# SymbioticLab/Oobleck

Measured on AMD Instinct MI355X. Metric: tokens/sec (whole node) GPT-2 1F1B, higher is better.
Workload: dtype bf16; 1 GPU; gpt2.yaml GPT-2-small 1F1B, global microbatch 128x1024 tokens, bf16; model=gpt2, global_batch=128, seq_len=1024, parallelism=pp1dp1

## Files before the change

include/oobleck_stage.h:

```cpp
#ifndef OOBLECK_STAGE_H
#define OOBLECK_STAGE_H

#include <stdint.h>

#ifdef __cplusplus
extern "C" {
#endif

enum {
  OB_KIND_EMBED = 0,
  OB_KIND_BLOCK = 1,
  OB_KIND_FINAL = 2
};

typedef struct ob_layer* ob_layer_t;

typedef struct {
  int32_t kind;
  int32_t n_embd;
  int32_t n_head;
  int32_t n_positions;
  int32_t vocab_size;
  int32_t max_batch;
  int32_t seq_len;
// ... 96 lines not shown
                    void* stream);
int ob_dropout_scale_f32(uint64_t seed, int32_t layer_id, int32_t site,
                         uint64_t tick, float p, const void* x, void* y,
                         int64_t n, void* stream);
int ob_dropout_scale_bf16(uint64_t seed, int32_t layer_id, int32_t site,
                          uint64_t tick, float p, const void* x, void* y,
                          int64_t n, void* stream);
int ob_dropout_add_f32(uint64_t seed, int32_t layer_id, int32_t site,
                       uint64_t tick, float p, const void* t, const void* res,
                       void* y, int64_t n, void* stream);
int ob_dropout_add_bf16(uint64_t seed, int32_t layer_id, int32_t site,
                        uint64_t tick, float p, const void* t,
                        const void* res, void* y, int64_t n, void* stream);
int ob_dropout_scale_colsum_f32(uint64_t seed, int32_t layer_id, int32_t site,
                                uint64_t tick, float p, const void* dy,
                                void* dm, void* db, int64_t M, int64_t N,
                                void* stream);
int ob_dropout_scale_colsum_bf16(uint64_t seed, int32_t layer_id, int32_t site,
                                 uint64_t tick, float p, const void* dy,
                                 void* dm, void* db, int64_t M, int64_t N,
                                 void* stream);

int ob_gemm_bf16(int transA, int transB, int64_t M, int64_t N, int64_t K,
                 float alpha, const void* A, int64_t lda,
                 int64_t strideA1, int64_t strideA2,
                 const void* B, int64_t ldb,
                 int64_t strideB1, int64_t strideB2,
                 float beta, void* C, int64_t ldc,
                 int64_t strideC1, int64_t strideC2,
                 int64_t n1, int64_t n2,
                 const void* bias, const void* residual, int out_kind,
                 int splitk, void* stream);

int ob_f32_to_bf16(const void* x, void* y, int64_t n, void* stream);
int ob_f32_to_bf16_t(const void* x, void* y, int64_t rows, int64_t cols,
                     void* stream);
int ob_bf16_to_f32(const void* x, void* y, int64_t n, void* stream);

void ob_profile_enable(int on);
void ob_profile_reset(void);
int ob_profile_read(int fam, double* total_ms, long long* count);

const char* ob_last_error(void);

const char* ob_build_arch(void);

#ifdef __cplusplus
}
#endif
#endif
```

oobleck_amd/_ext.py:

```python
from __future__ import annotations

import ctypes
import pathlib

_LIB = None
SO_PATH = pathlib.Path(__file__).resolve().parent / "libob_stage.so"


class ObLayerDesc(ctypes.Structure):
    _fields_ = [
        ("kind", ctypes.c_int32),
        ("n_embd", ctypes.c_int32),
        ("n_head", ctypes.c_int32),
        ("n_positions", ctypes.c_int32),
        ("vocab_size", ctypes.c_int32),
        ("max_batch", ctypes.c_int32),
        ("seq_len", ctypes.c_int32),
        ("n_slots", ctypes.c_int32),
        ("dtype", ctypes.c_int32),
    ]


class ObDropoutDesc(ctypes.Structure):
    _fields_ = [
# ... 78 lines not shown
    lib.ob_gemm_lt_bias.argtypes = [i32, i32, i64, i64, i64, f32, vp, i64,
                                    vp, i64, f32, vp, i64, i32, vp, vp]
    lib.ob_gemm_lt_f32.argtypes = [i32, i32, i64, i64, i64, f32, vp, i64,
                                   vp, i64, f32, vp, i64, vp]
    lib.ob_flash_fwd_bf16.argtypes = [vp, vp, vp, vp, i64, i64, i64, i64,
                                      f32, vp]
    lib.ob_transpose_bf16_b.argtypes = [vp, vp, i64, i64, i64, i64, i64,
                                        i64, i64, vp]
    lib.ob_layernorm_fwd_bf16.argtypes = [vp, vp, vp, vp, vp, vp, i64, i64,
                                          f32, vp]
    lib.ob_layernorm_bwd_bf16.argtypes = [vp, vp, vp, vp, vp, vp, vp, vp,
                                          i64, i64, i32, vp]
    lib.ob_colsum_bf16.argtypes = [vp, vp, i64, i64, vp]
    lib.ob_layernorm_fwd_copy_bf16.argtypes = [vp, vp, vp, vp, vp, vp, vp,
                                               i64, i64, f32, vp]
    lib.ob_layernorm_bwd_res_bf16.argtypes = [vp, vp, vp, vp, vp, vp, vp, vp,
                                              vp, vp, vp, i64, i64, vp]
    lib.ob_gelu_bwd_colsum_bf16.argtypes = [vp, vp, vp, vp, i64, i64, vp]
    lib.ob_gemm_lt.argtypes = [i32, i32, i64, i64, i64, f32, vp, i64, vp,
                               i64, f32, vp, i64, i32, vp]
    lib.ob_gemm_bf16_nt_8ph.argtypes = [vp, vp, vp, vp, vp, i64, i64, i64,
                                        i64, i64, i64, i64, i64, i64, i64,
                                        i64, i64, i64, i64, f32, f32, i32,
                                        i32, vp, i64]
    lib.ob_profile_enable.argtypes = [i32]
    lib.ob_profile_enable.restype = None
    lib.ob_profile_reset.argtypes = []
    lib.ob_profile_reset.restype = None
    lib.ob_profile_read.argtypes = [i32, ctypes.POINTER(ctypes.c_double),
                                    ctypes.POINTER(ctypes.c_longlong)]
    lib.ob_flash_dsum_bf16.argtypes = [vp, vp, vp, i64, i64, i64, i64, vp]
    lib.ob_flash_bwd_bf16.argtypes = [vp, vp, vp, vp, vp, vp, vp, vp, i64,
                                      i64, i64, i64, f32, vp]
    return lib


def get_ext(build_if_missing: bool = True) -> ctypes.CDLL:
    global _LIB
    if _LIB is not None:
        return _LIB
    if not SO_PATH.exists():
        if build_if_missing:
            from .build import build
            try:
                build()
            except Exception as e:
                raise RuntimeError(
                    f"oobleck_amd: HIP extension missing and build failed: {e}. "
                    "The hot path has no fallback — run __graft_entry__.build().") from e
        else:
            raise RuntimeError(
                "oobleck_amd: HIP extension libob_stage.so is missing. "
                "The hot path has no fallback — run __graft_entry__.build().")
    _LIB = _configure(ctypes.CDLL(str(SO_PATH)))
    return _LIB


def check(rc: int, what: str = "") -> None:
    if rc != 0:
        err = get_ext().ob_last_error().decode()
        raise RuntimeError(f"oobleck_amd extension error in {what}: {err}")
```

oobleck_amd/csrc/ob_internal.h:

```cpp
#pragma once
#include <hip/hip_runtime.h>

#include <cstdarg>
#include <cstdint>
#include <cstdio>

#include "../../include/oobleck_stage.h"

int ob_fail(const char* fmt, ...);

#define OB_HIP(x)                                                     \
  do {                                                                \
    hipError_t e_ = (x);                                              \
    if (e_ != hipSuccess)                                             \
      return ob_fail("%s:%d: %s", __FILE__, __LINE__,                 \
                     hipGetErrorString(e_));                          \
  } while (0)

#define OB_LAUNCH_CHECK()                                             \
  do {                                                                \
    hipError_t e_ = hipGetLastError();                                \
    if (e_ != hipSuccess)                                             \
      return ob_fail("%s:%d: launch: %s", __FILE__, __LINE__,         \
                     hipGetErrorString(e_));                          \
// ... 95 lines not shown
int ob_softmax_causal_bwd_bf16(const void* P, void* dP, int64_t batch,
                               int64_t Sq, void* stream);
int ob_gelu_fwd_bf16(const void* u, void* g, int64_t n, void* stream);
int ob_gelu_bwd_bf16(const void* u, const void* dg, void* du, int64_t n,
                     void* stream);
int ob_colsum_bf16(const void* X, void* db, int64_t M, int64_t N,
                   void* stream);
int ob_embed_fwd_bf16(const void* ids, const void* wte, const void* wpe,
                      void* out, int64_t B, int64_t Sq, int64_t H,
                      void* stream);
int ob_embed_bwd_bf16(const void* ids, const void* dout, void* dwte,
                      void* dwpe, int64_t B, int64_t Sq, int64_t H,
                      void* stream);
int ob_ce_fwd_bf16(const void* logits, const void* labels, void* lse,
                   void* loss, int64_t B, int64_t Sq, int64_t V, int64_t ld,
                   void* stream);
int ob_ce_bwd_bf16(void* logits, const void* labels, const void* lse,
                   const void* dloss, int64_t B, int64_t Sq, int64_t V,
                   int64_t ld, void* stream);
int ob_transpose_bf16(const void* in, void* out, int64_t R, int64_t C,
                      void* stream);
int ob_flash_fwd_bf16(const void* qkv, const void* VT, void* O, void* lse,
                      int64_t B, int64_t Sq, int64_t H, int64_t nh,
                      float scale, void* stream);
int ob_transpose_bf16_b(const void* in, void* out, int64_t R, int64_t C,
                        int64_t sIn1, int64_t sIn2, int64_t ldin, int64_t n1,
                        int64_t n2, void* stream);
int ob_flash_dsum_bf16(const void* O, const void* dO, void* D, int64_t B,
                       int64_t Sq, int64_t H, int64_t nh, void* stream);
int ob_flash_bwd_bf16(const void* qkv, const void* QT, const void* KT,
                      const void* dOT, const void* dO, const void* lse,
                      const void* D, void* dqkv, int64_t B, int64_t Sq,
                      int64_t H, int64_t nh, float scale, void* stream);
}
extern "C" int ob_gemm_lt(int tA, int tB, int64_t M, int64_t N, int64_t K,
                          float alpha, const void* A, int64_t lda,
                          const void* B, int64_t ldb, float beta, void* C,
                          int64_t ldc, int c_f32, void* stream);
extern "C" int ob_gemm_lt_bias(int tA, int tB, int64_t M, int64_t N,
                               int64_t K, float alpha, const void* A,
                               int64_t lda, const void* B, int64_t ldb,
                               float beta, void* C, int64_t ldc, int c_f32,
                               const void* bias, void* stream);
extern "C" int ob_gemm_lt_bias_res(int tA, int tB, int64_t M, int64_t N,
                                   int64_t K, float alpha, const void* A,
                                   int64_t lda, const void* B, int64_t ldb,
                                   void* C, int64_t ldc, int c_f32,
                                   const void* bias, const void* residual,
                                   void* stream);
extern "C" int ob_gemm_lt_f32(int tA, int tB, int64_t M, int64_t N,
                              int64_t K, float alpha, const void* A,
                              int64_t lda, const void* B, int64_t ldb,
                              float beta, void* C, int64_t ldc,
                              void* stream);
extern "C" int ob_gemm_bf16_nt_8ph(const void* A, const void* B, void* C,
                                   const void* bias, const void* residual,
                                   int64_t M, int64_t N, int64_t K,
                                   int64_t lda, int64_t ldb, int64_t ldc,
                                   int64_t sA1, int64_t sA2, int64_t sB1,
                                   int64_t sB2, int64_t sC1, int64_t sC2,
                                   int64_t n1, int64_t n2, float alpha,
                                   float beta, int out_kind, int splitk,
                                   void* stream, int64_t Mr);
int ob_gemm_bf16_nt_dispatch(const void* A, const void* B, void* C,
                             const void* bias, const void* residual,
                             int64_t M, int64_t N, int64_t K, int64_t lda,
// ... 6 lines not shown
```

oobleck_amd/csrc/ob_kernels_bf16.hip:

```cpp
#include "ob_internal.h"

#include <cmath>

using f32x16 = __attribute__((ext_vector_type(16))) float;
using bf16x8 = __attribute__((ext_vector_type(8))) __bf16;

static inline hipStream_t S(void* s) { return reinterpret_cast<hipStream_t>(s); }

#define BF_BM 128
#define BF_BN 128
#define BF_BK 32
#define BF_LDS_K 40

enum { BF_OUT_BF16 = 0, BF_OUT_F32 = 1, BF_OUT_F32_ATOMIC = 2 };

__device__ __forceinline__ float bf2f(__bf16 h) { return (float)h; }

__device__ __forceinline__ unsigned bf_bits(__bf16 h) {
  return (unsigned)__builtin_bit_cast(unsigned short, h);
}
__device__ __forceinline__ __bf16 bits_bf(unsigned u) {
  return __builtin_bit_cast(__bf16, (unsigned short)(u & 0xffffu));
}

// ... 3360 lines not shown
        (const __bf16*)qkv, (const __bf16*)QT, (const __bf16*)dOT,
        (const __bf16*)dO, (const float*)lse, (const float*)D,
        (__bf16*)dqkv, (int)Sq, (int)H, (int)nh, scale);
    OB_LAUNCH_CHECK();
  } else if (dsel == 'p') {
    dim3 gridp((unsigned)(Sq / 64), 1, (unsigned)(B * nh));
    k_flash_bwd_dkdv_p<<<gridp, 256, 0, S(stream)>>>(
        (const __bf16*)qkv, (const __bf16*)QT, (const __bf16*)dOT,
        (const __bf16*)dO, (const float*)lse, (const float*)D,
        (__bf16*)dqkv, (int)Sq, (int)H, (int)nh, scale);
    OB_LAUNCH_CHECK();
  } else {
    k_flash_bwd_dkdv<2><<<grid, 256, 0, S(stream)>>>(
        (const __bf16*)qkv, (const __bf16*)QT, (const __bf16*)dOT,
        (const __bf16*)dO, (const float*)lse, (const float*)D, (__bf16*)dqkv,
        (int)Sq, (int)H, (int)nh, scale);
    OB_LAUNCH_CHECK();
  }
  const char* dqe = getenv("OB_FLASH_DQ");
  if (dqe && dqe[0] == '1')
    k_flash_bwd_dq<<<grid, 256, 0, S(stream)>>>(
        (const __bf16*)qkv, (const __bf16*)KT, (const __bf16*)dO,
        (const float*)lse, (const float*)D, (__bf16*)dqkv, (int)Sq, (int)H,
        (int)nh, scale);
  else
    k_flash_bwd_dq_v3<<<grid, 256, 0, S(stream)>>>(
        (const __bf16*)qkv, (const __bf16*)KT, (const __bf16*)dO,
        (const float*)lse, (const float*)D, (__bf16*)dqkv, (int)Sq, (int)H,
        (int)nh, scale);
  OB_LAUNCH_CHECK();
  return 0;
}


using f32x4 = __attribute__((ext_vector_type(4))) float;

template <int OUT, int SWZ = 0>
__global__ __launch_bounds__(512, 1) void k_gemm_bf16_nt_8ph(
    const __bf16* __restrict__ A, const __bf16* __restrict__ B,
    void* __restrict__ Cv, const float* __restrict__ bias,
    const __bf16* __restrict__ R, int M, int N, int K, int64_t lda,
    int64_t ldb, int64_t ldc, int64_t sA1, int64_t sA2, int64_t sB1,
    int64_t sB2, int64_t sC1, int64_t sC2, int n2, float alpha, float beta,
    int nbn, int Mr) {
  __shared__ __bf16 lds[2][4][128 * 64];

  const int tile = bf_xcd_swz(blockIdx.x, gridDim.x);
  const int bm = tile / nbn, bn = tile % nbn;
  const int m0 = bm * 256, n0 = bn * 256;

  const int z = blockIdx.z;
  const int i1 = z / n2, i2 = z % n2;
  A += (int64_t)i1 * sA1 + (int64_t)i2 * sA2;
  B += (int64_t)i1 * sB1 + (int64_t)i2 * sB2;
  float* Cf = reinterpret_cast<float*>(Cv);
  __bf16* Cb = reinterpret_cast<__bf16*>(Cv);
  const int64_t coff = (int64_t)i1 * sC1 + (int64_t)i2 * sC2;
  Cf += coff;
  Cb += coff;
  if (R) R += coff;

  const int splitk = gridDim.y;
  constexpr int BK = 64;
  const int kchunk = ((K + splitk * BK - 1) / (splitk * BK)) * BK;
  const int kbeg = blockIdx.y * kchunk;
  const int kend = min(K, kbeg + kchunk);
// ... 195 lines not shown
```

oobleck_amd/csrc/ob_layer.hip:

```cpp
#include "ob_internal.h"
#include "ob_philox.h"

#include <cmath>
#include <cstring>
#include <vector>

static inline hipStream_t S(void* s) { return reinterpret_cast<hipStream_t>(s); }
static inline int64_t i64min(int64_t a, int64_t b) { return a < b ? a : b; }
static inline int64_t i64max(int64_t a, int64_t b) { return a > b ? a : b; }


struct Workspace {
  float* dp = nullptr;
  float* bsh1 = nullptr;
  float* bsh2 = nullptr;
  float* dqkv = nullptr;
  float* b4h = nullptr;
  float* t1 = nullptr;
  float* t2 = nullptr;
  float* s1 = nullptr;
  float* s2 = nullptr;
  float* pd_f = nullptr;
  float* pd_b = nullptr;
  float* dm1 = nullptr;
// ... 125 lines not shown
  int64_t o_x = 0, o_mean1 = 0, o_rstd1 = 0, o_ln1 = 0, o_qkv = 0, o_p = 0,
          o_attnm = 0, o_hmid = 0, o_mean2 = 0, o_rstd2 = 0, o_ln2 = 0,
          o_u = 0, o_g = 0, o_logits = 0, o_lse = 0;
  __bf16* shadows = nullptr;
  int64_t v_pad = 0;
  int64_t sh_qkv = 0, sh_qkv_t = 0, sh_ap = 0, sh_ap_t = 0, sh_fc = 0,
          sh_fc_t = 0, sh_mp = 0, sh_mp_t = 0, sh_lm = 0, sh_lm_t = 0;
  int64_t shadow_count = 0;
  bool flash = false;
  float p_embd = 0.f, p_resid = 0.f, p_attn = 0.f;
  int32_t layer_id = 0;
  uint64_t seed = 0;
  bool training = true;
  uint64_t next_tick = 0;
  std::vector<uint8_t> slot_drop;
  std::vector<uint64_t> slot_tick;
};

static bool has_dropout(const ob_layer* l) {
  return l->p_embd > 0.f || l->p_resid > 0.f || l->p_attn > 0.f;
}
static ob_drop_key drop_key(const ob_layer* l, int slot, int site, float p) {
  return ob_drop_make_key(l->seed, l->layer_id, site, l->slot_tick[slot], p);
}

static bool flash_eligible(const ob_layer_desc* d, float attn_pdrop = 0.f) {
  if (attn_pdrop > 0.f) return false;
  static const bool off = [] {
    const char* e = getenv("OB_BF16_FLASH");
    return e && e[0] == '0';
  }();
  return !off && d->dtype == 1 && d->n_embd / d->n_head == 64 &&
         d->seq_len % 128 == 0;
}

struct BlockParams {
  int64_t ln1_w, ln1_b, w_qkv, b_qkv, w_attnproj, b_attnproj, ln2_w, ln2_b,
      w_fc, b_fc, w_mlpproj, b_mlpproj, total;
};
static BlockParams block_params(int64_t H) {
  BlockParams p;
  int64_t o = 0;
  p.ln1_w = o; o += H;
  p.ln1_b = o; o += H;
  p.w_qkv = o; o += H * 3 * H;
  p.b_qkv = o; o += 3 * H;
  p.w_attnproj = o; o += H * H;
  p.b_attnproj = o; o += H;
  p.ln2_w = o; o += H;
  p.ln2_b = o; o += H;
  p.w_fc = o; o += H * 4 * H;
  p.b_fc = o; o += 4 * H;
  p.w_mlpproj = o; o += 4 * H * H;
  p.b_mlpproj = o; o += H;
  p.total = o;
  return p;
}

extern "C" int64_t ob_layer_param_count(const ob_layer_desc* d) {
  const int64_t H = d->n_embd, V = d->vocab_size, P = d->n_positions;
  switch (d->kind) {
    case OB_KIND_EMBED: return V * H + P * H;
    case OB_KIND_BLOCK: return block_params(H).total;
    case OB_KIND_FINAL: return 2 * H + V * H;
  }
  return -1;
// ... 78 lines not shown
      return ob_fail("create: ids hipMalloc failed");
    }
  }
  l->v_pad = (V + 255) / 256 * 256;
  if (d->dtype == 1) {
    int64_t o2 = 0;
    if (d->kind == OB_KIND_BLOCK) {
      l->sh_qkv = o2; o2 += 3 * H * H;
      l->sh_qkv_t = o2; o2 += 3 * H * H;
      l->sh_ap = o2; o2 += H * H;
      l->sh_ap_t = o2; o2 += H * H;
      l->sh_fc = o2; o2 += 4 * H * H;
      l->sh_fc_t = o2; o2 += 4 * H * H;
      l->sh_mp = o2; o2 += 4 * H * H;
      l->sh_mp_t = o2; o2 += 4 * H * H;
    } else if (d->kind == OB_KIND_FINAL) {
      l->sh_lm = o2; o2 += l->v_pad * H;
      l->sh_lm_t = o2; o2 += H * l->v_pad;
    }
    l->shadow_count = o2;
    if (o2 > 0) {
      if (hipMalloc(&l->shadows, (size_t)o2 * sizeof(__bf16)) != hipSuccess)
        return ob_fail("create: shadow hipMalloc failed");
      OB_HIP(hipMemset(l->shadows, 0, (size_t)o2 * sizeof(__bf16)));
    }
  }
  if (d->kind == OB_KIND_BLOCK) {
    if (!l->flash &&
        ws_ensure(&g_ws.dp, &g_ws.sz_dp, Bm * nh * Sq * Sq))
      return 1;
    if (ws_ensure(&g_ws.dqkv, &g_ws.sz_dqkv, BS * 3 * H)) return 1;
    if (ws_ensure(&g_ws.b4h, &g_ws.sz_b4h, BS * 4 * H)) return 1;
    if (d->dtype == 1) {
      if (ws_ensure(&g_ws.t1, &g_ws.sz_t1, (4 * H * BS + 1) / 2)) return 1;
      if (ws_ensure(&g_ws.t2, &g_ws.sz_t2, (4 * H * BS + 1) / 2)) return 1;
      if (ws_ensure(&g_ws.s1, &g_ws.sz_s1, (4 * H * BS + 1) / 2)) return 1;
      if (ws_ensure(&g_ws.s2, &g_ws.sz_s2, (4 * H * BS + 1) / 2)) return 1;
      if (side_init()) return 1;
    }
  }
  if (d->kind == OB_KIND_FINAL && d->dtype == 1) {
    if (ws_ensure(&g_ws.t1, &g_ws.sz_t1, (l->v_pad * BS + 1) / 2)) return 1;
    if (ws_ensure(&g_ws.t2, &g_ws.sz_t2, (4 * H * BS + 1) / 2)) return 1;
    if (ws_ensure(&g_ws.s1, &g_ws.sz_s1, (l->v_pad * BS + 1) / 2)) return 1;
    if (ws_ensure(&g_ws.s2, &g_ws.sz_s2, (4 * H * BS + 1) / 2)) return 1;
    if (side_init()) return 1;
  }
  if (d->kind != OB_KIND_EMBED) {
    const int64_t need = BSH;
    if (ws_ensure(&g_ws.bsh1, &g_ws.sz_bsh, need)) return 1;
    if (ws_ensure(&g_ws.bsh2, &g_ws.sz_bsh2, need)) return 1;
  }
  if (l->p_attn > 0.f) {
    if (ws_ensure(&g_ws.pd_f, &g_ws.sz_pd_f, Bm * nh * Sq * Sq)) return 1;
    if (ws_ensure(&g_ws.pd_b, &g_ws.sz_pd_b, Bm * nh * Sq * Sq)) return 1;
  }
  if (l->p_resid > 0.f) {
    if (ws_ensure(&g_ws.dm1, &g_ws.sz_dm1, BSH)) return 1;
    if (ws_ensure(&g_ws.dm2, &g_ws.sz_dm2, BSH)) return 1;
  }
  *out = l;
  return 0;
}

extern "C" int ob_layer_create(const ob_layer_desc* d, ob_layer_t* out) {
  return layer_create(d, nullptr, out);
}

// ... 267 lines not shown
  return gemm_bf(0, 1, actw, dyw, BS, 1.f, XT, BS, 0, 0, DYT, BS, 0, 0, gout,
                 ldc, 0, 0, 1, 1, nullptr, nullptr, 2,
                 pick_splitk(actw, dyw, BS), stream);
}

static bool use_flash(const ob_layer* l) { return l->flash; }

static int block_forward_bf16(ob_layer* l, int slot, const __bf16* in,
                              __bf16* out, void* stream) {
  const int64_t Sq = l->d.seq_len, H = l->d.n_embd, nh = l->d.n_head;
  const int64_t B = l->B, BS = B * Sq;
  const int64_t hd = H / nh;
  float* st = l->stash + (int64_t)slot * l->slot_stride;
  const float* p = l->params;
  const __bf16* sh = l->shadows;
  const BlockParams bp = block_params(H);
  const bool dA = l->slot_drop[slot] && l->p_attn > 0.f;
  const bool dR = l->slot_drop[slot] && l->p_resid > 0.f;

  __bf16* x = (__bf16*)(st + l->o_x);
  __bf16* ln1 = (__bf16*)(st + l->o_ln1);
  if (OB_PROF(OB_PF_LN, stream,
              ob_layernorm_fwd_copy_bf16(in, p + bp.ln1_w, p + bp.ln1_b, ln1,
                                         x, st + l->o_mean1, st + l->o_rstd1,
                                         BS, H, 1e-5f, stream)))
    return 1;
  __bf16* qkv = (__bf16*)(st + l->o_qkv);
  if (OB_PROF(OB_PF_GEMM_FWD, stream,
              gemm_bf(0, 1, BS, 3 * H, H, 1.f, ln1, H, 0, 0,
                      sh + l->sh_qkv_t, H, 0, 0, qkv, 3 * H, 0, 0, 1, 1,
                      p + bp.b_qkv, nullptr, 0, 1, stream)))
    return 1;
  __bf16* am = (__bf16*)(st + l->o_attnm);
  if (use_flash(l)) {
    __bf16* VTw = (__bf16*)g_ws.t2;
    if (OB_PROF(OB_PF_FLASH_FWD, stream,
                ob_transpose_bf16_b(qkv + 2 * H, VTw, Sq, 64, Sq * 3 * H, 64,
                                    3 * H, B, nh, stream)))
      return 1;
    float* lseP = st + l->o_p;
    if (OB_PROF(OB_PF_FLASH_FWD, stream,
                ob_flash_fwd_bf16(qkv, VTw, am, lseP, B, Sq, H, nh,
                                  1.f / sqrtf((float)hd), stream)))
      return 1;
  } else {
    __bf16* P = (__bf16*)(st + l->o_p);
    if (OB_PROF(OB_PF_ATTN_MAT, stream,
                gemm_bf(0, 1, Sq, Sq, hd, 1.f, qkv, 3 * H, Sq * 3 * H, hd,
                        qkv + H, 3 * H, Sq * 3 * H, hd, P, Sq, nh * Sq * Sq,
                        Sq * Sq, B, nh, nullptr, nullptr, 0, 1, stream)))
      return 1;
    if (OB_PROF(OB_PF_ATTN_MAT, stream,
                ob_softmax_causal_fwd_bf16(P, B * nh, Sq,
                                           1.f / sqrtf((float)hd), stream)))
      return 1;
    const __bf16* Pv = P;
    if (dA) {
      if (OB_PROF(OB_PF_ELEM, stream,
                  ob_drop_scale(drop_key(l, slot, OB_DROP_ATTN, l->p_attn), 1,
                                P, g_ws.pd_f, B * nh * Sq * Sq, stream)))
        return 1;
      Pv = (const __bf16*)g_ws.pd_f;
    }
    if (OB_PROF(OB_PF_ATTN_MAT, stream,
                gemm_bf(0, 0, Sq, hd, Sq, 1.f, Pv, Sq, nh * Sq * Sq, Sq * Sq,
                        qkv + 2 * H, 3 * H, Sq * 3 * H, hd, am, H, Sq * H,
                        hd, B, nh, nullptr, nullptr, 0, 1, stream)))
// ... 137 lines not shown
              gemm_bf(0, 1, BS, H, 4 * H, 1.f, DY4, 4 * H, 0, 0,
                      sh + l->sh_fc, 4 * H, 0, 0, DLN, H, 0, 0, 1, 1,
                      nullptr, nullptr, 0, 1, stream)))
    return 1;
  if (OB_PROF(OB_PF_LN, stream,
              ob_layernorm_bwd_res_bf16(hmid, p + bp.ln2_w, st + l->o_mean2,
                                        st + l->o_rstd2, DLN, dout, din,
                                        g + bp.ln2_w, g + bp.ln2_b,
                                        dR ? nullptr : g + bp.b_mlpproj,
                                        dR ? nullptr : g + bp.b_attnproj,
                                        BS, H, stream)))
    return 1;
  const __bf16* dap = din;
  if (dR) {
    if (OB_PROF(OB_PF_ELEM, stream,
                ob_drop_scale_colsum(
                    drop_key(l, slot, OB_DROP_RESID_ATTN, l->p_resid), 1, din,
                    g_ws.dm1, g + bp.b_attnproj, BS, H, stream)))
      return 1;
    dap = (const __bf16*)g_ws.dm1;
  }
  OB_SIDE_FENCE(S(stream), g_side.stream);
  if (OB_PROF(OB_PF_GEMM_DX, stream,
              gemm_bf(0, 1, BS, H, H, 1.f, dap, H, 0, 0, sh + l->sh_ap, H, 0,
                      0, DATT, H, 0, 0, 1, 1, nullptr, nullptr, 0, 1,
                      stream)))
    return 1;
  if (OB_PROF(OB_PF_GEMM_DW, side,
              dw_bf16_ws(am, H, dap, H, BS, g + bp.w_attnproj, H, g_ws.s1,
                         g_ws.s2, side)))
    return 1;
  hipEvent_t ev_din_done = side_evt();
  OB_HIP(hipEventRecord(ev_din_done, g_side.stream));
  if (use_flash(l)) {
    const int64_t BSH = BS * H;
    __bf16* QTw = (__bf16*)g_ws.t1;
    __bf16* KTw = QTw + BSH;
    __bf16* dOTw = KTw + BSH;
    float* Dbuf = g_ws.t1 + (3 * BSH + 1) / 2;
    const float* lseP = st + l->o_p;
    if (OB_PROF(OB_PF_FLASH_BWD, stream,
                ob_transpose_bf16_b(qkv, QTw, Sq, 64, Sq * 3 * H, 64, 3 * H,
                                    B, nh, stream)))
      return 1;
    if (OB_PROF(OB_PF_FLASH_BWD, stream,
                ob_transpose_bf16_b(qkv + H, KTw, Sq, 64, Sq * 3 * H, 64,
                                    3 * H, B, nh, stream)))
      return 1;
    if (OB_PROF(OB_PF_FLASH_BWD, stream,
                ob_transpose_bf16_b(DATT, dOTw, Sq, 64, Sq * H, 64, H, B, nh,
                                    stream)))
      return 1;
    if (OB_PROF(OB_PF_FLASH_BWD, stream,
                ob_flash_dsum_bf16(am, DATT, Dbuf, B, Sq, H, nh, stream)))
      return 1;
    if (OB_PROF(OB_PF_FLASH_BWD, stream,
                ob_flash_bwd_bf16(qkv, QTw, KTw, dOTw, DATT, lseP, Dbuf,
                                  DQKV, B, Sq, H, nh, scale, stream)))
      return 1;
  } else {
    if (OB_PROF(OB_PF_ATTN_MAT, stream,
                gemm_bf(0, 1, Sq, Sq, hd, 1.f, DATT, H, Sq * H, hd,
                        qkv + 2 * H, 3 * H, Sq * 3 * H, hd, DP, Sq,
                        nh * Sq * Sq, Sq * Sq, B, nh, nullptr, nullptr, 0, 1,
                        stream)))
      return 1;
    const __bf16* Pv = P;
    if (dA) {
      const ob_drop_key ka = drop_key(l, slot, OB_DROP_ATTN, l->p_attn);
      if (OB_PROF(OB_PF_ELEM, stream,
                  ob_drop_scale(ka, 1, P, g_ws.pd_b, B * nh * Sq * Sq,
                                stream)))
        return 1;
      if (OB_PROF(OB_PF_ELEM, stream,
                  ob_drop_scale(ka, 1, DP, DP, B * nh * Sq * Sq, stream)))
        return 1;
      Pv = (const __bf16*)g_ws.pd_b;
    }
    if (OB_PROF(OB_PF_ATTN_MAT, stream,
                ob_softmax_causal_bwd_bf16(P, DP, B * nh, Sq, stream)))
      return 1;
    if (OB_PROF(OB_PF_ATTN_MAT, stream,
                gemm_bf(0, 0, Sq, hd, Sq, scale, DP, Sq, nh * Sq * Sq,
                        Sq * Sq, qkv + H, 3 * H, Sq * 3 * H, hd, DQKV, 3 * H,
                        Sq * 3 * H, hd, B, nh, nullptr, nullptr, 0, 1,
                        stream)))
      return 1;
    if (OB_PROF(OB_PF_ATTN_MAT, stream,
                gemm_bf(1, 0, Sq, hd, Sq, scale, DP, Sq, nh * Sq * Sq,
                        Sq * Sq, qkv, 3 * H, Sq * 3 * H, hd, DQKV + H, 3 * H,
                        Sq * 3 * H, hd, B, nh, nullptr, nullptr, 0, 1,
                        stream)))
      return 1;
    if (OB_PROF(OB_PF_ATTN_MAT, stream,
                gemm_bf(1, 0, Sq, hd, Sq, 1.f, Pv, Sq, nh * Sq * Sq, Sq * Sq,
                        DATT, H, Sq * H, hd, DQKV + 2 * H, 3 * H, Sq * 3 * H,
                        hd, B, nh, nullptr, nullptr, 0, 1, stream)))
      return 1;
  }
  OB_SIDE_FENCE(S(stream), g_side.stream);
  if (OB_PROF(OB_PF_ELEM, side,
              ob_colsum_bf16(DQKV, g + bp.b_qkv, BS, 3 * H, side)))
    return 1;
  if (OB_PROF(OB_PF_GEMM_DW, side,
              dw_bf16_ws(ln1, H, DQKV, 3 * H, BS, g + bp.w_qkv, 3 * H,
                         g_ws.s1, g_ws.s2, side)))
    return 1;
  if (OB_PROF(OB_PF_GEMM_DX, stream,
              gemm_bf(0, 1, BS, H, 3 * H, 1.f, DQKV, 3 * H, 0, 0,
                      sh + l->sh_qkv, 3 * H, 0, 0, DLN, H, 0, 0, 1, 1,
                      nullptr, nullptr, 0, 1, stream)))
    return 1;
  OB_HIP(hipStreamWaitEvent(S(stream), ev_din_done, 0));
  if (OB_PROF(OB_PF_LN, stream,
              ob_layernorm_bwd_bf16(x, p + bp.ln1_w, st + l->o_mean1,
                                    st + l->o_rstd1, DLN, din, g + bp.ln1_w,
                                    g + bp.ln1_b, BS, H, 1, stream)))
    return 1;
  OB_SIDE_FENCE(g_side.stream, S(stream));
  return 0;
}

static int final_backward_bf16(ob_layer* l, int slot, const float* dout,
                               __bf16* din, void* stream) {
  const int64_t Sq = l->d.seq_len, H = l->d.n_embd, V = l->d.vocab_size;
  const int64_t B = l->B, BS = B * Sq;
  float* st = l->stash + (int64_t)slot * l->slot_stride;
  const float* p = l->params;
  float* g = l->grads;
  __bf16* x = (__bf16*)(st + l->o_x);
  __bf16* lnf = (__bf16*)(st + l->o_ln1);
  __bf16* logits = (__bf16*)(st + l->o_logits);
  int64_t* labs = l->ids + (int64_t)slot * (int64_t)l->d.max_batch * Sq;
  __bf16* DLN = (__bf16*)g_ws.bsh1;
// ... 275 lines not shown
```

Before: 639,300 tokens/s.

## Add transpose-free flash attention kernels using LDS transposed reads and fused qkv bias grad

Adds new flash attention forward and backward kernels that read Q, K and V straight from the packed qkv buffer. They stage tiles in swizzled LDS and use ds_read_tr16 transposed loads, so the separate transpose kernels for V, Q, K and dO are no longer needed. The backward kernels also fold the qkv bias gradient column-sum into their epilogues through atomics, which drops the separate colsum launch. The path is on by default and can be turned off with an environment variable. In exchange it adds float atomics on the bias gradient and rebalances the backward work between a dK/dV kernel and a dQ kernel.

```diff
diff --git a/include/oobleck_stage.h b/include/oobleck_stage.h
--- a/include/oobleck_stage.h
+++ b/include/oobleck_stage.h
@@ -152,6 +152,14 @@
                  const void* bias, const void* residual, int out_kind,
                  int splitk, void* stream);
 
+int ob_flash_fwd_nt_bf16(const void* qkv, void* O, void* lse, int64_t B,
+                         int64_t Sq, int64_t H, int64_t nh, float scale,
+                         void* stream);
+int ob_flash_bwd_nt_bf16(const void* qkv, const void* dO, const void* lse,
+                         const void* D, void* dqkv, void* dbias_qkv,
+                         int64_t B, int64_t Sq, int64_t H, int64_t nh,
+                         float scale, void* stream);
+
 int ob_f32_to_bf16(const void* x, void* y, int64_t n, void* stream);
 int ob_f32_to_bf16_t(const void* x, void* y, int64_t rows, int64_t cols,
                      void* stream);
diff --git a/oobleck_amd/_ext.py b/oobleck_amd/_ext.py
--- a/oobleck_amd/_ext.py
+++ b/oobleck_amd/_ext.py
@@ -134,6 +134,10 @@
     lib.ob_flash_dsum_bf16.argtypes = [vp, vp, vp, i64, i64, i64, i64, vp]
     lib.ob_flash_bwd_bf16.argtypes = [vp, vp, vp, vp, vp, vp, vp, vp, i64,
                                       i64, i64, i64, f32, vp]
+    lib.ob_flash_fwd_nt_bf16.argtypes = [vp, vp, vp, i64, i64, i64, i64,
+                                         f32, vp]
+    lib.ob_flash_bwd_nt_bf16.argtypes = [vp, vp, vp, vp, vp, vp, i64, i64,
+                                         i64, i64, f32, vp]
     return lib
 
 
diff --git a/oobleck_amd/csrc/ob_internal.h b/oobleck_amd/csrc/ob_internal.h
--- a/oobleck_amd/csrc/ob_internal.h
+++ b/oobleck_amd/csrc/ob_internal.h
@@ -151,6 +151,13 @@
                       const void* dOT, const void* dO, const void* lse,
                       const void* D, void* dqkv, int64_t B, int64_t Sq,
                       int64_t H, int64_t nh, float scale, void* stream);
+int ob_flash_fwd_nt_bf16(const void* qkv, void* O, void* lse, int64_t B,
+                         int64_t Sq, int64_t H, int64_t nh, float scale,
+                         void* stream);
+int ob_flash_bwd_nt_bf16(const void* qkv, const void* dO, const void* lse,
+                         const void* D, void* dqkv, void* dbias_qkv,
+                         int64_t B, int64_t Sq, int64_t H, int64_t nh,
+                         float scale, void* stream);
 }
 extern "C" int ob_gemm_lt(int tA, int tB, int64_t M, int64_t N, int64_t K,
                           float alpha, const void* A, int64_t lda,
diff --git a/oobleck_amd/csrc/ob_kernels_bf16.hip b/oobleck_amd/csrc/ob_kernels_bf16.hip
--- a/oobleck_amd/csrc/ob_kernels_bf16.hip
+++ b/oobleck_amd/csrc/ob_kernels_bf16.hip
@@ -3416,6 +3416,472 @@
   return 0;
 }
 
+using bf16x4 = __attribute__((ext_vector_type(4))) __bf16;
+
+__device__ __forceinline__ int nt_key(int row) {
+  return (((row >> 1) & 1) << 2) | ((row >> 2) & 3);
+}
+__device__ __forceinline__ int nt_off(int row, int ch) {
+  return row * 64 + ((ch ^ nt_key(row)) << 3);
+}
+__device__ __forceinline__ bf16x8 nt_tr_frag(const __bf16* tile, int lane,
+                                             int r0, int dhalf) {
+  typedef __attribute__((address_space(3))) bf16x4 lds_bf16x4;
+  const int i = lane & 15;
+  const int row = r0 + (i >> 2);
+  const int ch = 4 * dhalf + 2 * ((lane >> 4) & 1) + ((i >> 1) & 1);
+  const int sub = 4 * (i & 1);
+  const bf16x4 lo = __builtin_amdgcn_ds_read_tr16_b64_v4bf16(
+      (lds_bf16x4*)(tile + nt_off(row, ch) + sub));
+  const bf16x4 hi = __builtin_amdgcn_ds_read_tr16_b64_v4bf16(
+      (lds_bf16x4*)(tile + nt_off(row + 4, ch) + sub));
+  return __builtin_shufflevector(lo, hi, 0, 1, 2, 3, 4, 5, 6, 7);
+}
+
+__global__ __launch_bounds__(256, 3) void k_flash_fwd_nt(
+    const __bf16* __restrict__ qkv, __bf16* __restrict__ Obase,
+    float* __restrict__ lse, int Sq, int H, int nh, float scale) {
+  __shared__ __attribute__((aligned(16))) __bf16 kbuf[2][64 * 64];
+  __shared__ __attribute__((aligned(16))) __bf16 vbuf[2][64 * 64];
+  __shared__ float bcast[128];
+  const int z = blockIdx.z;
+  const int b = z / nh, h = z % nh;
+  const int64_t qoff = (int64_t)b * Sq * 3 * H + h * 64;
+  const __bf16* Qp = qkv + qoff;
+  const __bf16* Kp = Qp + H;
+  const __bf16* Vp = Qp + 2 * H;
+  __bf16* Op = Obase + (int64_t)b * Sq * H + h * 64;
+  float* lsep = lse + (int64_t)z * Sq;
+
+  const int tid = threadIdx.x;
+  const int lane = tid & 63;
+  const int w = tid >> 6;
+  const int il = lane & 31, kh = lane >> 5;
+  const int q0b = blockIdx.x * 128;
+  const int q0 = q0b + w * 32;
+  const int myq = q0 + il;
+
+  const int sr0 = tid >> 3, sr1 = sr0 + 32, sc = tid & 7;
+  const int so0 = nt_off(sr0, sc), so1 = nt_off(sr1, sc);
+  auto stage = [&](int buf, int kv0) {
+    *reinterpret_cast<bf16x8*>(&kbuf[buf][so0]) =
+        *reinterpret_cast<const bf16x8*>(
+            Kp + (int64_t)(kv0 + sr0) * 3 * H + sc * 8);
+    *reinterpret_cast<bf16x8*>(&kbuf[buf][so1]) =
+        *reinterpret_cast<const bf16x8*>(
+            Kp + (int64_t)(kv0 + sr1) * 3 * H + sc * 8);
+    *reinterpret_cast<bf16x8*>(&vbuf[buf][so0]) =
+        *reinterpret_cast<const bf16x8*>(
+            Vp + (int64_t)(kv0 + sr0) * 3 * H + sc * 8);
+    *reinterpret_cast<bf16x8*>(&vbuf[buf][so1]) =
+        *reinterpret_cast<const bf16x8*>(
+            Vp + (int64_t)(kv0 + sr1) * 3 * H + sc * 8);
+  };
+
+  bf16x8 qf[4];
+#pragma unroll
+  for (int s = 0; s < 4; ++s)
+    qf[s] = *reinterpret_cast<const bf16x8*>(
+        Qp + (int64_t)myq * 3 * H + s * 16 + kh * 8);
+
+  const int ntiles = (q0b + 128) / 64;
+  stage(0, 0);
+  __syncthreads();
+
+  f32x16 o0 = {}, o1 = {};
+  float m = -INFINITY, l = 0.f;
+  for (int kvt = 0; kvt < ntiles; ++kvt) {
+    const int kv0 = kvt * 64;
+    if (kvt + 1 < ntiles) stage((kvt + 1) & 1, kv0 + 64);
+    const bool active = kv0 <= q0 + 31;
+    if (active) {
+      const __bf16* kb = kbuf[kvt & 1];
+      const __bf16* vb = vbuf[kvt & 1];
+      f32x16 sacc0 = {}, sacc1 = {};
+#pragma unroll
+      for (int s = 0; s < 4; ++s) {
+        const int ch = (s * 2 + kh);
+        const bf16x8 ka =
+            *reinterpret_cast<const bf16x8*>(&kb[nt_off(il, ch)]);
+        const bf16x8 kb2 =
+            *reinterpret_cast<const bf16x8*>(&kb[nt_off(32 + il, ch)]);
+        sacc0 = __builtin_amdgcn_mfma_f32_32x32x16_bf16(ka, qf[s], sacc0, 0,
+                                                        0, 0);
+        sacc1 = __builtin_amdgcn_mfma_f32_32x32x16_bf16(kb2, qf[s], sacc1,
+                                                        0, 0, 0);
+      }
+      float sv[32];
+      if (kv0 + 63 < q0) {
+#pragma unroll
+        for (int r = 0; r < 16; ++r) {
+          sv[r] = sacc0[r] * scale;
+          sv[16 + r] = sacc1[r] * scale;
+        }
+      } else {
+#pragma unroll
+        for (int r = 0; r < 16; ++r) {
+          const int kvr = kv0 + (r & 3) + 8 * (r >> 2) + 4 * kh;
+          sv[r] = (kvr <= myq) ? sacc0[r] * scale : -INFINITY;
+          sv[16 + r] = (kvr + 32 <= myq) ? sacc1[r] * scale : -INFINITY;
+        }
+      }
+      float mx[8];
+#pragma unroll
+      for (int j = 0; j < 8; ++j)
+        mx[j] = fmaxf(fmaxf(sv[j], sv[8 + j]),
+                      fmaxf(sv[16 + j], sv[24 + j]));
+      float mt = fmaxf(fmaxf(fmaxf(mx[0], mx[1]), fmaxf(mx[2], mx[3])),
+                       fmaxf(fmaxf(mx[4], mx[5]), fmaxf(mx[6], mx[7])));
+      mt = fmaxf(mt, __shfl_xor(mt, 32, 64));
+      const bool rescale = !__all(mt - m <= 8.f);
+      if (rescale) {
+        const float mnew = fmaxf(m, mt);
+        const float af = __expf(m - mnew);
+        m = mnew;
+        if (kh == 0) bcast[w * 32 + il] = af;
+#pragma unroll
+        for (int r = 0; r < 16; ++r) {
+          const float a = bcast[w * 32 + (r & 3) + 8 * (r >> 2) + 4 * kh];
+          o0[r] *= a;
+          o1[r] *= a;
+        }
+        l *= af;
+      }
+      float ps[8] = {};
+#pragma unroll
+      for (int r = 0; r < 32; ++r) {
+        sv[r] = (sv[r] == -INFINITY) ? 0.f : __expf(sv[r] - m);
+        ps[r & 7] += sv[r];
+      }
+      float psum = ((ps[0] + ps[1]) + (ps[2] + ps[3])) +
+                   ((ps[4] + ps[5]) + (ps[6] + ps[7]));
+      psum += __shfl_xor(psum, 32, 64);
+      l += psum;
+#pragma unroll
+      for (int t = 0; t < 4; ++t) {
+        const bf16x8 pa = bf_dance(sv + t * 8);
+        const bf16x8 v0f = nt_tr_frag(vb, lane, t * 16 + kh * 8, 0);
+        const bf16x8 v1f = nt_tr_frag(vb, lane, t * 16 + kh * 8, 1);
+        o0 = __builtin_amdgcn_mfma_f32_32x32x16_bf16(pa, v0f, o0, 0, 0, 0);
+        o1 = __builtin_amdgcn_mfma_f32_32x32x16_bf16(pa, v1f, o1, 0, 0, 0);
+      }
+    }
+    __syncthreads();
+  }
+
+  if (kh == 0) {
+    bcast[w * 32 + il] = 1.f / l;
+    lsep[myq] = m + __logf(l);
+  }
+#pragma unroll
+  for (int r = 0; r < 16; ++r) {
+    const int row = (r & 3) + 8 * (r >> 2) + 4 * kh;
+    const float inv = bcast[w * 32 + row];
+    Op[(int64_t)(q0 + row) * H + il] = (__bf16)(o0[r] * inv);
+    Op[(int64_t)(q0 + row) * H + 32 + il] = (__bf16)(o1[r] * inv);
+  }
+}
+
+extern "C" int ob_flash_fwd_nt_bf16(const void* qkv, void* O, void* lse,
+                                    int64_t B, int64_t Sq, int64_t H,
+                                    int64_t nh, float scale, void* stream) {
+  if (H / nh != 64) return ob_fail("flash_fwd_nt: head_dim must be 64");
+  if (Sq % 128) return ob_fail("flash_fwd_nt: S must be a multiple of 128");
+  dim3 grid((unsigned)(Sq / 128), 1, (unsigned)(B * nh));
+  k_flash_fwd_nt<<<grid, 256, 0, S(stream)>>>(
+      (const __bf16*)qkv, (__bf16*)O, (float*)lse, (int)Sq, (int)H, (int)nh,
+      scale);
+  OB_LAUNCH_CHECK();
+  return 0;
+}
+
+__global__ __launch_bounds__(256, 3) void k_flash_bwd_dkdv_nt(
+    const __bf16* __restrict__ qkv, const __bf16* __restrict__ dO,
+    const float* __restrict__ lse, const float* __restrict__ D,
+    __bf16* __restrict__ dqkv, float* __restrict__ dbias, int Sq, int H,
+    int nh, float scale) {
+  __shared__ float xch[2][2][32 * 32];
+  __shared__ __attribute__((aligned(16))) __bf16 qbuf[2][32 * 64];
+  __shared__ __attribute__((aligned(16))) __bf16 obuf[2][32 * 64];
+  __shared__ float red[4 * 64];
+  const int z = blockIdx.z;
+  const int b = z / nh, h = z % nh;
+  const int64_t base = (int64_t)b * Sq * 3 * H + h * 64;
+  const __bf16* Qp = qkv + base;
+  const __bf16* Kp = Qp + H;
+  const __bf16* Vp = Qp + 2 * H;
+  const __bf16* dOp = dO + (int64_t)b * Sq * H + h * 64;
+  const float* lsep = lse + (int64_t)z * Sq;
+  const float* Dp = D + (int64_t)z * Sq;
+
+  const int tid = threadIdx.x;
+  const int lane = tid & 63;
+  const int w = tid >> 6;
+  const int pair = w >> 1, role = w & 1;
+  const int il = lane & 31, kh = lane >> 5;
+  const int kv0 = blockIdx.x * 64 + pair * 32;
+  const int mykv = kv0 + il;
+
+  const __bf16* KV = role ? Vp : Kp;
+  bf16x8 of[4];
+#pragma unroll
+  for (int s = 0; s < 4; ++s)
+    of[s] = *reinterpret_cast<const bf16x8*>(
+        KV + (int64_t)mykv * 3 * H + s * 16 + kh * 8);
+
+  const int srow = tid >> 3, schunk = tid & 7;
+  const int so = nt_off(srow, schunk);
+  auto stage = [&](int buf, int q0s) {
+    *reinterpret_cast<bf16x8*>(&qbuf[buf][so]) =
+        *reinterpret_cast<const bf16x8*>(
+            Qp + (int64_t)(q0s + srow) * 3 * H + schunk * 8);
+    *reinterpret_cast<bf16x8*>(&obuf[buf][so]) =
+        *reinterpret_cast<const bf16x8*>(
+            dOp + (int64_t)(q0s + srow) * H + schunk * 8);
+  };
+
+  f32x16 acc0 = {}, acc1 = {};
+  const int nqt = Sq / 32;
+  const int qt0 = (blockIdx.x * 64) / 32;
+  stage(qt0 & 1, qt0 * 32);
+  __syncthreads();
+
+  for (int qt = qt0; qt < nqt; ++qt) {
+    const int q0 = qt * 32;
+    if (qt + 1 < nqt) stage((qt + 1) & 1, q0 + 32);
+    const __bf16* ab = role ? obuf[qt & 1] : qbuf[qt & 1];
+    const __bf16* bb = role ? qbuf[qt & 1] : obuf[qt & 1];
+    const bf16x8 b00 = nt_tr_frag(bb, lane, kh * 8, 0);
+    const bf16x8 b01 = nt_tr_frag(bb, lane, kh * 8, 1);
+    const bf16x8 b10 = nt_tr_frag(bb, lane, 16 + kh * 8, 0);
+    const bf16x8 b11 = nt_tr_frag(bb, lane, 16 + kh * 8, 1);
+    f32x16 own = {};
+#pragma unroll
+    for (int s = 0; s < 4; ++s) {
+      const int ch = s * 2 + kh;
+      const bf16x8 af =
+          *reinterpret_cast<const bf16x8*>(&ab[nt_off(il, ch)]);
+      own = __builtin_amdgcn_mfma_f32_32x32x16_bf16(af, of[s], own, 0, 0,
+                                                    0);
+    }
+    float pv[16];
+    float* ptile = xch[qt & 1][pair];
+    if (role == 0) {
+      const float lse_t = lsep[q0 + il];
+#pragma unroll
+      for (int r = 0; r < 16; ++r) {
+        const int qoff = acc_row(r, kh);
+        const bool ok = q0 + qoff >= mykv;
+        const float lse_q = __shfl(lse_t, qoff, 64);
+        pv[r] = ok ? __expf(own[r] * scale - lse_q) : 0.f;
+        ptile[qoff * 32 + il] = pv[r];
+      }
+    }
+    __syncthreads();
+    if (role == 1) {
+      const float d_t = Dp[q0 + il];
+#pragma unroll
+      for (int r = 0; r < 16; ++r) {
+        const int qoff = acc_row(r, kh);
+        const float d_q = __shfl(d_t, qoff, 64);
+        pv[r] = ptile[qoff * 32 + il] * (own[r] - d_q);
+      }
+    }
+#pragma unroll
+    for (int t = 0; t < 2; ++t) {
+      const bf16x8 a = bf_dance(pv + t * 8);
+      const bf16x8 bl = t ? b10 : b00;
+      const bf16x8 bh = t ? b11 : b01;
+      acc0 = __builtin_amdgcn_mfma_f32_32x32x16_bf16(a, bl, acc0, 0, 0, 0);
+      acc1 = __builtin_amdgcn_mfma_f32_32x32x16_bf16(a, bh, acc1, 0, 0, 0);
+    }
+  }
+
+  __bf16* outp = dqkv + base + (role ? H : 2 * H);
+  const float os = role ? scale : 1.f;
+#pragma unroll
+  for (int r = 0; r < 16; ++r) {
+    const int kv = kv0 + acc_row(r, kh);
+    outp[(int64_t)kv * 3 * H + il] = (__bf16)(os * acc0[r]);
+    outp[(int64_t)kv * 3 * H + 32 + il] = (__bf16)(os * acc1[r]);
+  }
+  if (dbias) {
+    float c0 = 0.f, c1 = 0.f;
+#pragma unroll
+    for (int r = 0; r < 16; ++r) {
+      c0 += os * acc0[r];
+      c1 += os * acc1[r];
+    }
+    c0 += __shfl_xor(c0, 32, 64);
+    c1 += __shfl_xor(c1, 32, 64);
+    if (kh == 0) {
+      red[w * 64 + il] = c0;
+      red[w * 64 + 32 + il] = c1;
+    }
+    __syncthreads();
+    if (tid < 128) {
+      const int rl = tid >> 6, c = tid & 63;
+      atomicAdd(dbias + (rl ? H : 2 * H) + h * 64 + c,
+                red[rl * 64 + c] + red[(2 + rl) * 64 + c]);
+    }
+  }
+}
+
+__global__ __launch_bounds__(256, 3) void k_flash_bwd_dq_nt(
+    const __bf16* __restrict__ qkv, const __bf16* __restrict__ dO,
+    const float* __restrict__ lse, const float* __restrict__ D,
+    __bf16* __restrict__ dqkv, float* __restrict__ dbias, int Sq, int H,
+    int nh, float scale) {
+  __shared__ __attribute__((aligned(16))) __bf16 kbuf[2][64 * 64];
+  __shared__ __attribute__((aligned(16))) __bf16 vbuf[2][64 * 64];
+  __shared__ float red[4 * 64];
+  const int z = blockIdx.z;
+  const int b = z / nh, h = z % nh;
+  const int64_t base = (int64_t)b * Sq * 3 * H + h * 64;
+  const __bf16* Qp = qkv + base;
+  const __bf16* Kp = Qp + H;
+  const __bf16* Vp = Qp + 2 * H;
+  const __bf16* dOp = dO + (int64_t)b * Sq * H + h * 64;
+  const float* lsep = lse + (int64_t)z * Sq;
+  const float* Dp = D + (int64_t)z * Sq;
+
+  const int tid = threadIdx.x;
+  const int lane = tid & 63;
+  const int w = tid >> 6;
+  const int il = lane & 31, kh = lane >> 5;
+  const int q0 = blockIdx.x * 128 + w * 32;
+  const int myq = q0 + il;
+  const float mylse = lsep[myq];
+  const float myD = Dp[myq];
+
+  bf16x8 qf[4], df[4];
+#pragma unroll
+  for (int s = 0; s < 4; ++s) {
+    qf[s] = *reinterpret_cast<const bf16x8*>(
+        Qp + (int64_t)myq * 3 * H + s * 16 + kh * 8);
+    df[s] = *reinterpret_cast<const bf16x8*>(
+        dOp + (int64_t)myq * H + s * 16 + kh * 8);
+  }
+
+  const int srow = tid >> 3, schunk = tid & 7;
+  const int so0 = nt_off(srow, schunk), so1 = nt_off(srow + 32, schunk);
+  auto stage = [&](int buf, int kv0) {
+    *reinterpret_cast<bf16x8*>(&kbuf[buf][so0]) =
+        *reinterpret_cast<const bf16x8*>(
+            Kp + (int64_t)(kv0 + srow) * 3 * H + schunk * 8);
+    *reinterpret_cast<bf16x8*>(&kbuf[buf][so1]) =
+        *reinterpret_cast<const bf16x8*>(
+            Kp + (int64_t)(kv0 + srow + 32) * 3 * H + schunk * 8);
+    *reinterpret_cast<bf16x8*>(&vbuf[buf][so0]) =
+        *reinterpret_cast<const bf16x8*>(
+            Vp + (int64_t)(kv0 + srow) * 3 * H + schunk * 8);
+    *reinterpret_cast<bf16x8*>(&vbuf[buf][so1]) =
+        *reinterpret_cast<const bf16x8*>(
+            Vp + (int64_t)(kv0 + srow + 32) * 3 * H + schunk * 8);
+  };
+
+  const int ntiles = (blockIdx.x * 128 + 128) / 64;
+  stage(0, 0);
+  __syncthreads();
+
+  f32x16 dq0 = {}, dq1 = {};
+  for (int kvt = 0; kvt < ntiles; ++kvt) {
+    const int kv0 = kvt * 64;
+    if (kvt + 1 < ntiles) stage((kvt + 1) & 1, kv0 + 64);
+    const bool active = kv0 <= q0 + 31;
+    if (active) {
+      const __bf16* kb = kbuf[kvt & 1];
+      const __bf16* vb = vbuf[kvt & 1];
+      f32x16 s0 = {}, s1 = {}, p0 = {}, p1 = {};
+#pragma unroll
+      for (int s = 0; s < 4; ++s) {
+        const int ch = s * 2 + kh;
+        const bf16x8 ka =
+            *reinterpret_cast<const bf16x8*>(&kb[nt_off(il, ch)]);
+        const bf16x8 kb2 =
+            *reinterpret_cast<const bf16x8*>(&kb[nt_off(32 + il, ch)]);
+        const bf16x8 va =
+            *reinterpret_cast<const bf16x8*>(&vb[nt_off(il, ch)]);
+        const bf16x8 vb2 =
+            *reinterpret_cast<const bf16x8*>(&vb[nt_off(32 + il, ch)]);
+        s0 = __builtin_amdgcn_mfma_f32_32x32x16_bf16(ka, qf[s], s0, 0, 0, 0);
+        s1 = __builtin_amdgcn_mfma_f32_32x32x16_bf16(kb2, qf[s], s1, 0, 0,
+                                                     0);
+        p0 = __builtin_amdgcn_mfma_f32_32x32x16_bf16(va, df[s], p0, 0, 0, 0);
+        p1 = __builtin_amdgcn_mfma_f32_32x32x16_bf16(vb2, df[s], p1, 0, 0,
+                                                     0);
+      }
+      float dsv[32];
+#pragma unroll
+      for (int r = 0; r < 16; ++r) {
+        const int kv = kv0 + (r & 3) + 8 * (r >> 2) + 4 * kh;
+        const bool ok0 = kv <= myq;
+        const bool ok1 = kv + 32 <= myq;
+        const float pa = ok0 ? __expf(s0[r] * scale - mylse) : 0.f;
+        const float pb = ok1 ? __expf(s1[r] * scale - mylse) : 0.f;
+        dsv[r] = ok0 ? pa * (p0[r] - myD) : 0.f;
+        dsv[16 + r] = ok1 ? pb * (p1[r] - myD) : 0.f;
+      }
+#pragma unroll
+      for (int t = 0; t < 4; ++t) {
+        const bf16x8 da = bf_dance(dsv + t * 8);
+        const bf16x8 kt0 = nt_tr_frag(kb, lane, t * 16 + kh * 8, 0);
+        const bf16x8 kt1 = nt_tr_frag(kb, lane, t * 16 + kh * 8, 1);
+        dq0 = __builtin_amdgcn_mfma_f32_32x32x16_bf16(da, kt0, dq0, 0, 0, 0);
+        dq1 = __builtin_amdgcn_mfma_f32_32x32x16_bf16(da, kt1, dq1, 0, 0, 0);
+      }
+    }
+    __syncthreads();
+  }
+  __bf16* dQp = dqkv + base;
+#pragma unroll
+  for (int r = 0; r < 16; ++r) {
+    const int q = q0 + (r & 3) + 8 * (r >> 2) + 4 * kh;
+    dQp[(int64_t)q * 3 * H + il] = (__bf16)(scale * dq0[r]);
+    dQp[(int64_t)q * 3 * H + 32 + il] = (__bf16)(scale * dq1[r]);
+  }
+  if (dbias) {
+    float c0 = 0.f, c1 = 0.f;
+#pragma unroll
+    for (int r = 0; r < 16; ++r) {
+      c0 += scale * dq0[r];
+      c1 += scale * dq1[r];
+    }
+    c0 += __shfl_xor(c0, 32, 64);
+    c1 += __shfl_xor(c1, 32, 64);
+    if (kh == 0) {
+      red[w * 64 + il] = c0;
+      red[w * 64 + 32 + il] = c1;
+    }
+    __syncthreads();
+    if (tid < 64)
+      atomicAdd(dbias + h * 64 + tid, (red[tid] + red[64 + tid]) +
+                                          (red[128 + tid] + red[192 + tid]));
+  }
+}
+
+extern "C" int ob_flash_bwd_nt_bf16(const void* qkv, const void* dO,
+                                    const void* lse, const void* D,
+                                    void* dqkv, void* dbias_qkv, int64_t B,
+                                    int64_t Sq, int64_t H, int64_t nh,
+                                    float scale, void* stream) {
+  if (H / nh != 64) return ob_fail("flash_bwd_nt: head_dim must be 64");
+  if (Sq % 128) return ob_fail("flash_bwd_nt: S must be a multiple of 128");
+  dim3 gridp((unsigned)(Sq / 64), 1, (unsigned)(B * nh));
+  k_flash_bwd_dkdv_nt<<<gridp, 256, 0, S(stream)>>>(
+      (const __bf16*)qkv, (const __bf16*)dO, (const float*)lse,
+      (const float*)D, (__bf16*)dqkv, (float*)dbias_qkv, (int)Sq, (int)H,
+      (int)nh, scale);
+  OB_LAUNCH_CHECK();
+  dim3 grid((unsigned)(Sq / 128), 1, (unsigned)(B * nh));
+  k_flash_bwd_dq_nt<<<grid, 256, 0, S(stream)>>>(
+      (const __bf16*)qkv, (const __bf16*)dO, (const float*)lse,
+      (const float*)D, (__bf16*)dqkv, (float*)dbias_qkv, (int)Sq, (int)H,
+      (int)nh, scale);
+  OB_LAUNCH_CHECK();
+  return 0;
+}
+
 
 using f32x4 = __attribute__((ext_vector_type(4))) float;
 
diff --git a/oobleck_amd/csrc/ob_layer.hip b/oobleck_amd/csrc/ob_layer.hip
--- a/oobleck_amd/csrc/ob_layer.hip
+++ b/oobleck_amd/csrc/ob_layer.hip
@@ -181,6 +181,14 @@
   }();
   return !off && d->dtype == 1 && d->n_embd / d->n_head == 64 &&
          d->seq_len % 128 == 0;
+}
+
+static bool flash_tr() {
+  static const bool on = [] {
+    const char* e = getenv("OB_FLASH_TR");
+    return !(e && e[0] == '0');
+  }();
+  return on;
 }
 
 struct BlockParams {
@@ -325,8 +333,12 @@
     if (ws_ensure(&g_ws.dqkv, &g_ws.sz_dqkv, BS * 3 * H)) return 1;
     if (ws_ensure(&g_ws.b4h, &g_ws.sz_b4h, BS * 4 * H)) return 1;
     if (d->dtype == 1) {
-      if (ws_ensure(&g_ws.t1, &g_ws.sz_t1, (4 * H * BS + 1) / 2)) return 1;
-      if (ws_ensure(&g_ws.t2, &g_ws.sz_t2, (4 * H * BS + 1) / 2)) return 1;
+      if (l->flash && flash_tr()) {
+        if (ws_ensure(&g_ws.t1, &g_ws.sz_t1, Bm * nh * Sq)) return 1;
+      } else {
+        if (ws_ensure(&g_ws.t1, &g_ws.sz_t1, (4 * H * BS + 1) / 2)) return 1;
+        if (ws_ensure(&g_ws.t2, &g_ws.sz_t2, (4 * H * BS + 1) / 2)) return 1;
+      }
       if (ws_ensure(&g_ws.s1, &g_ws.sz_s1, (4 * H * BS + 1) / 2)) return 1;
       if (ws_ensure(&g_ws.s2, &g_ws.sz_s2, (4 * H * BS + 1) / 2)) return 1;
       if (side_init()) return 1;
@@ -660,7 +672,13 @@
                       p + bp.b_qkv, nullptr, 0, 1, stream)))
     return 1;
   __bf16* am = (__bf16*)(st + l->o_attnm);
-  if (use_flash(l)) {
+  if (use_flash(l) && flash_tr()) {
+    float* lseP = st + l->o_p;
+    if (OB_PROF(OB_PF_FLASH_FWD, stream,
+                ob_flash_fwd_nt_bf16(qkv, am, lseP, B, Sq, H, nh,
+                                     1.f / sqrtf((float)hd), stream)))
+      return 1;
+  } else if (use_flash(l)) {
     __bf16* VTw = (__bf16*)g_ws.t2;
     if (OB_PROF(OB_PF_FLASH_FWD, stream,
                 ob_transpose_bf16_b(qkv + 2 * H, VTw, Sq, 64, Sq * 3 * H, 64,
@@ -864,7 +882,19 @@
     return 1;
   hipEvent_t ev_din_done = side_evt();
   OB_HIP(hipEventRecord(ev_din_done, g_side.stream));
-  if (use_flash(l)) {
+  const bool flash_nt = use_flash(l) && flash_tr();
+  if (flash_nt) {
+    float* Dbuf = g_ws.t1;
+    const float* lseP = st + l->o_p;
+    if (OB_PROF(OB_PF_FLASH_BWD, stream,
+                ob_flash_dsum_bf16(am, DATT, Dbuf, B, Sq, H, nh, stream)))
+      return 1;
+    if (OB_PROF(OB_PF_FLASH_BWD, stream,
+                ob_flash_bwd_nt_bf16(qkv, DATT, lseP, Dbuf, DQKV,
+                                     g + bp.b_qkv, B, Sq, H, nh, scale,
+                                     stream)))
+      return 1;
+  } else if (use_flash(l)) {
     const int64_t BSH = BS * H;
     __bf16* QTw = (__bf16*)g_ws.t1;
     __bf16* KTw = QTw + BSH;
@@ -931,7 +961,8 @@
       return 1;
   }
   OB_SIDE_FENCE(S(stream), g_side.stream);
-  if (OB_PROF(OB_PF_ELEM, side,
+  if (!flash_nt &&
+      OB_PROF(OB_PF_ELEM, side,
               ob_colsum_bf16(DQKV, g + bp.b_qkv, BS, 3 * H, side)))
     return 1;
   if (OB_PROF(OB_PF_GEMM_DW, side,
```

New measurement: 667,200 tokens/s (median of 6 runs). 1.04x the previous value.
